# schreibfaul1/ESP32-Opus-Player

Measured on AMD Instinct MI355X. Metric: decoded 48 kHz stereo frames/sec/GPU (x real-time); HBM GB/s vs roofline, higher is better.
Workload: dtype int32 fixed-point (int16/int32 with 64-bit products); 1 GPU; celt_fb_stereo_64k; streams_per_gpu=65536

## Files before the change

esp32-opus-player_amd/csrc/og_celt.hpp:

```cpp
#pragma once
#include "og_celt_bands.hpp"

namespace og {

struct WaveArr {
    typedef RomGlobal Rom;
    OG_MEMBER i32 &pulses(int i) const { return S.pulses_row()[i]; }
    OG_MEMBER i32 &alloc_bits(int i) const { return S.pulses_row()[i]; }
    OG_MEMBER void pulses_rest(int, int) const {}
    OG_MEMBER i32 &fine_quant(int i) const { return S.fine_quant[i]; }
    OG_MEMBER i32 &fine_prio(int i) const { return S.fine_prio[i]; }
    OG_MEMBER i32 &tf_res(int i) const { return S.tf_res[i]; }
    OG_MEMBER void boost_put(int i, int n, int quanta) const { S.offsets[i] = n * quanta; }
    OG_MEMBER i32 boost(int i, int, int) const { return S.offsets[i]; }
    OG_MEMBER i32 &bits1(int i) const { return S.bits1[i]; }
    OG_MEMBER i32 &bits2(int i) const { return S.bits2[i]; }
    OG_MEMBER i16 &bandE(int i) const { return S.bandE_row()[i]; }
    OG_MEMBER void energies_rest() const {}
    OG_MEMBER void energies_back() const {}
};

template <class A, class R>
OG_DEV void coarse_energy(A a, R &rc, int start, int end, int intra, int C, int LM) {
    typedef typename A::Rom T;
    const int pm = (LM * 2 + intra) * 42;
    i32 prev0 = 0, prev1 = 0;
    i32 coef, beta;
    if (intra) {
        coef = 0;
        beta = 4915;
    } else {
        beta = LM == 0 ? 30147 : LM == 1 ? 22282 : LM == 2 ? 12124 : 6554;
        coef = LM == 0 ? 29440 : LM == 1 ? 26112 : LM == 2 ? 21248 : 16384;
    }
    const i32 budget = (i32)rc.storage * 8;
    for (int i = start; i < end; i++) {
        for (int c = 0; c < C; c++) {
            int qi;
            i32 tell = rc_tell(rc);
            if (budget - tell >= 15) {
                int pi = 2 * OG_MIN(i, 20);
                qi = rc_laplace(rc, (u32)T::eprob(pm + pi) << 7, (int)T::eprob(pm + pi + 1) << 6);
            } else if (budget - tell >= 2) {
                u32 s = rc.rng, d = rc.val, r = s >> 2, t;
                int ret = -1;
                do {
                    t = s;
                    ++ret;
                    s = r * (u32)(2 - ret);
                } while (d < s);
                rc.val = d - s;
                rc.rng = t - s;
                rc_renorm(rc);
                qi = (ret >> 1) ^ -(ret & 1);
            } else if (budget - tell >= 1) {
                qi = -rc_bit_logp(rc, 1);
            } else
                qi = -1;
            i32 q = shl32(qi, 10);
            i32 e = OG_MAX(-9 * 1024, (i32)a.bandE(i + c * NBANDS));
            const i32 pv = c ? prev1 : prev0;
            i32 tmp = pshr32(mul16(coef, e), 8) + pv + shl32(q, 7);
            tmp = OG_MAX(-(28 << 17), tmp);
            a.bandE(i + c * NBANDS) = (i16)pshr32(tmp, 7);
            const i32 nv = pv + shl32(q, 7) - mul16(beta, pshr32(q, 8));
            if (c) prev1 = nv; else prev0 = nv;
        }
    }
}

template <class A, class R>
OG_DEV void fine_energy(A a, R &rc, int start, int end, int C) {
    for (int i = start; i < end; i++) {
        int fq = a.fine_quant(i);
        if (fq <= 0) continue;
        for (int c = 0; c < C; c++) {
            i32 q2 = (i32)rc_bits(rc, fq);
            i32 offset = tr16(sub16((shl32(q2, 10) + 512) >> fq, 512));
            a.bandE(i + c * NBANDS) = (i16)(a.bandE(i + c * NBANDS) + offset);
        }
    }
}

template <class A, class R>
OG_DEV void energy_finalise(A a, R &rc, int start, int end, int bits_left, int C) {
    for (int prio = 0; prio < 2; prio++) {
        for (int i = start; i < end && bits_left >= C; i++) {
            if (a.fine_quant(i) >= 8 || a.fine_prio(i) != prio) continue;
            for (int c = 0; c < C; c++) {
                i32 q2 = (i32)rc_bits(rc, 1);
                i32 offset = tr16((shl16(q2, 10) - 512) >> (a.fine_quant(i) + 1));
                a.bandE(i + c * NBANDS) = (i16)(a.bandE(i + c * NBANDS) + offset);
                bits_left--;
            }
        }
    }
}

OG_DEV int tf_select(int LM, int idx) {
    const u32 row0 = 0xF0F0F0F0u, row1 = 0xF101E0F0u, row2 = 0xF102D0E0u, row3 = 0xF103D0E0u;
    u32 row = LM == 0 ? row0 : LM == 1 ? row1 : LM == 2 ? row2 : row3;
    int v = (int)((row >> (4 * idx)) & 15);
    return v >= 8 ? v - 16 : v;
}

template <class A, class R>
OG_DEV void tf_decode(A a, R &rc, int start, int end, int transient, int LM) {
    int curr = 0, tf_sel = 0, tf_changed = 0;
    int logp = transient ? 2 : 4;
    u32 budget = rc.storage * 8, tell = (u32)rc_tell(rc);
    int rsv = LM > 0 && tell + logp + 1 <= budget;
    budget -= rsv;
    for (int i = start; i < end; i++) {
        if (tell + logp <= budget) {
            curr ^= rc_bit_logp(rc, logp);
            tell = (u32)rc_tell(rc);
            tf_changed |= curr;
        }
        a.tf_res(i) = curr;
        logp = transient ? 4 : 5;
    }
    if (rsv && tf_select(LM, 4 * transient + 0 + tf_changed) != tf_select(LM, 4 * transient + 2 + tf_changed))
        tf_sel = rc_bit_logp(rc, 1);
    for (int i = start; i < end; i++) a.tf_res(i) = tf_select(LM, 4 * transient + 2 * tf_sel + a.tf_res(i));
}

template <class T>
OG_DEV i32 celt_band_cap(int j, int LM, int C) {
    const int Nb = (T::eband(j + 1) - T::eband(j)) << LM;
    return (T::pulse_caps(NBANDS * (2 * LM + C - 1) + j) + 64) * C * Nb >> 2;
}

template <class T>
OG_DEV i32 dynalloc_quanta(int j, int LM, int C) {
    const int width = C * (T::eband(j + 1) - T::eband(j)) << LM;
    return OG_MIN(width << BITRES, OG_MAX(6 << BITRES, width));
}

template <class A, class R>
OG_DEV int compute_allocation(A a, R &rc, int start, int end, int alloc_trim, i32 &intensity, i32 &dual_stereo, i32 total,
                               i32 &balance_out, int C, int LM) {
    typedef typename A::Rom T;
    int skip_start = start, intensity_rsv = 0, dual_stereo_rsv = 0;
    OG_STAT(59, total < 0);
    total = OG_MAX(total, 0);
    int skip_rsv = total >= 1 << BITRES ? 1 << BITRES : 0;
    total -= skip_rsv;
    if (C == 2) {
        intensity_rsv = T::log2_frac(end - start);
        if (intensity_rsv > total)
            intensity_rsv = 0;
        else {
            total -= intensity_rsv;
            dual_stereo_rsv = total >= 1 << BITRES ? 1 << BITRES : 0;
// ... 1179 lines not shown
                      const i16 *__restrict__ silk, int silk_n) {
    const i32 t0 = s0 + m;
    m = mul16x32_q15(27853, t0);
    const i32 t1 = s1 + m;
    m = mul16x32_q15(27853, t1);
    const i32 t2 = s2 + m;
    m = mul16x32_q15(27853, t2);
    const i32 t3 = s3 + m;
    m = mul16x32_q15(27853, t3);
#ifdef OG_HOST_EMUL
    const i32 o0 = post_mix(sat16(pshr32(t0, 12)), silk, silk_n, (j + 0) * CC + c), o1 = post_mix(sat16(pshr32(t1, 12)), silk, silk_n, (j + 1) * CC + c);
    const i32 o2 = post_mix(sat16(pshr32(t2, 12)), silk, silk_n, (j + 2) * CC + c), o3 = post_mix(sat16(pshr32(t3, 12)), silk, silk_n, (j + 3) * CC + c);
#else
    const PostAdd ad = post_addends(silk, silk_n, j, c, CC);
    const i32 o0 = sat16(sat16(pshr32(t0, 12)) + ad.a0), o1 = sat16(sat16(pshr32(t1, 12)) + ad.a1);
    const i32 o2 = sat16(sat16(pshr32(t2, 12)) + ad.a2), o3 = sat16(sat16(pshr32(t3, 12)) + ad.a3);
#endif
#ifdef OG_HOST_EMUL
    if (pcm) {
        pcm[(j + 0) * CC + c] = (i16)o0;
        pcm[(j + 1) * CC + c] = (i16)o1;
        pcm[(j + 2) * CC + c] = (i16)o2;
        pcm[(j + 3) * CC + c] = (i16)o3;
    }
#else
    const u32 w01 = (u32)(u16)o0 | (u32)(u16)o1 << 16;
    const u32 w23 = (u32)(u16)o2 | (u32)(u16)o3 << 16;
    og_v2u out;
    int at;
    if (CC == 2) {
        const u32 p01 = (u32)__shfl_xor((int)w01, 1, 64), p23 = (u32)__shfl_xor((int)w23, 1, 64);
        if (c == 0) {
            out.x = (w01 & 0xffffu) | p01 << 16;
            out.y = w01 >> 16 | (p01 & 0xffff0000u);
        } else {
            out.x = (p23 & 0xffffu) | w23 << 16;
            out.y = p23 >> 16 | (w23 & 0xffff0000u);
        }
        at = (j + 2 * c) * 2;
    } else {
        out.x = w01;
        out.y = w23;
        at = j;
    }
    if (pcm) *reinterpret_cast<og_v2u *>(pcm + at) = out;
#endif
}

OG_DEV void celt_post_lane(CeltState *st, int c, int CC, int N, int pos, i16 *__restrict__ pcm, const i16 *__restrict__ silk, int silk_n) {
    const i32 *ring = st->ring[c];
    i32 m = st->deemph[c];
#ifdef OG_HOST_EMUL
    for (int j = 0; j < N; j += 4) {
        const i32 *src = &ring[(pos + j) & RING_MASK];
        celt_post4(m, src[0], src[1], src[2], src[3], j, c, CC, pcm, silk, silk_n);
    }
#else
#define OG_LD4(j) (*reinterpret_cast<const og_v4i *>(&ring[(pos + (j)) & RING_MASK]))
    og_v4i a0 = OG_LD4(0), a1 = OG_LD4(4), a2 = OG_LD4(8), a3 = OG_LD4(12);
    for (int j = 0; j < N; j += 16) {
        const int jn = j + 16 < N ? j + 16 : j;
        const og_v4i b0 = OG_LD4(jn), b1 = OG_LD4(jn + 4), b2 = OG_LD4(jn + 8), b3 = OG_LD4(jn + 12);
        celt_post4(m, a0.x, a0.y, a0.z, a0.w, j, c, CC, pcm, silk, silk_n);
        celt_post4(m, a1.x, a1.y, a1.z, a1.w, j + 4, c, CC, pcm, silk, silk_n);
        celt_post4(m, a2.x, a2.y, a2.z, a2.w, j + 8, c, CC, pcm, silk, silk_n);
        celt_post4(m, a3.x, a3.y, a3.z, a3.w, j + 12, c, CC, pcm, silk, silk_n);
        a0 = b0;
        a1 = b1;
        a2 = b2;
        a3 = b3;
    }
#undef OG_LD4
#endif
    st->deemph[c] = m;
}


OG_DEV void celt_synthesis(CeltState *st, const CeltSynth &p) {
    const int N = p.N, LM = p.LM, C = p.C, CC = p.CC, start = p.start, end = p.end, silence = p.silence, transient = p.transient;
    const int pf_pitch = p.pf_pitch, pf_tapset = p.pf_tapset, M = 1 << LM;
    const i32 pf_gain = p.pf_gain;
    denorm_gains(start, end, C, silence);
    OG_SYNC();
    if (C == 1) {
        OG_FOR_LANES(i, NBANDS) S.bandE_row()[NBANDS + i] = S.bandE_row()[i];
        OG_SYNC();
    }
    if (!p.lost) OG_FOR_LANES(i, 2 * NBANDS) {
        int band = i >= NBANDS ? i - NBANDS : i;
        i32 e = S.bandE_row()[i], l1 = S.logE1_row()[i], l2 = S.logE2_row()[i];
        if (!transient) {
            l2 = l1;
            l1 = e;
        } else
            l1 = OG_MIN(l1, e);
        if (p.loss && !transient) {
            const i32 inc = p.loss->celt_loss_count < 10 ? M : 1024;
            p.loss->backgroundLogE[i] = (i16)OG_MIN((i32)(i16)(p.loss->backgroundLogE[i] + inc), e);
        }
        if (band < start || band >= end) {
            e = 0;
            l1 = l2 = -28 * 1024;
        }
        if (!p.energies_kept_by_parse) st->bandE[i] = (i16)e;
        st->logE1[i] = (i16)l1;
        st->logE2[i] = (i16)l2;
    }
    const int B = transient ? M : 1, shift = transient ? 3 : 3 - LM;
    const int pp = OG_MAX(p.have_state ? p.st_pf_period : st->pf_period, 15), ppo = OG_MAX(p.have_state ? p.st_pf_period_old : st->pf_period_old, 15);
    const i32 pg = p.have_state ? p.st_pf_gain : st->pf_gain, pgo = p.have_state ? p.st_pf_gain_old : st->pf_gain_old;
    const int pt = p.have_state ? p.st_pf_tapset : st->pf_tapset, pto = p.have_state ? p.st_pf_tapset_old : st->pf_tapset_old;
    const int pos = p.have_state ? p.st_ring_pos : st->ring_pos;
    i32 *const SY = syn_buf();
#if defined(OG_RECON_TIGHT) && !defined(OG_HOST_EMUL)
    int touch_code = 0;
    if (!p.lost && LM != 0 && (pgo != 0 || pg != 0 || pf_gain != 0)) {
        const CombRun span = comb_touch_span(comb_touch_plan(ppo, pp, pf_pitch, pgo, pg, pf_gain, pto, pt, pf_tapset, N));
        if (span.lo <= span.hi) touch_code = comb_touch_code(span, pos);
    }
#endif
#ifdef OG_RECON_TIGHT
    for (int c = CC - 1; c >= 0; c--) {
#else
    for (int c = 0; c < CC; c++) {
#endif
        OG_SYNC();
        OG_MARK(14);
#if defined(OG_RECON_TIGHT) && !defined(OG_HOST_EMUL)
        if (!(CC == 1 && C == 2)) denorm_bins((CC == 2 && C == 1) ? 0 : c);
        imdct_channel(st->tail[c], c, N, LM, B, shift, C, CC, st->ring[c], touch_code);
#else
        imdct_channel(st->tail[c], c, N, LM, B, shift, C, CC);
#endif
        OG_MARK(15);
        OG_TAP(2 + 16 * c);
        if (!p.lost) {
            comb_filter(st, c, 0, ppo, pp, 120, pgo, pg, pto, pt, pos);
            if (LM != 0) comb_filter(st, c, 120, pp, pf_pitch, N - 120, pg, pf_gain, pt, pf_tapset, pos);
        }
        OG_TAP(3 + 16 * c);
        OG_SYNC();
        if (p.inline_deemph && OG_LANE == 0) {
            const int plane = pcm_plane(c, C, CC);
            i32 m = st->deemph[c];
            for (int j = 0; j < N; j++) {
                i32 tmp = SY[j] + m;
                m = mul16x32_q15(27853, tmp);
                S.v[plane + j] = (i16)sat16(pshr32(tmp, 12));
            }
            st->deemph[c] = m;
        }
        OG_SYNC();
        OG_MARK(16);
        OG_FOR_LANES(i, N) st->ring[c][(pos + i) & RING_MASK] = SY[i];
        OG_FOR_LANES(i, OVERLAP / 2) st->tail[c][i] = SY[N + i];
    }
    OG_SYNC();
    if (OG_LANE == 0 && p.lost) {
        st->ring_pos = (pos + N) & RING_MASK;
        st->rng = p.rng_final;
        p.loss->celt_loss_count += 1;
    } else if (OG_LANE == 0) {
        if (p.loss) p.loss->celt_loss_count = 0;
        st->ring_pos = (pos + N) & RING_MASK;
        st->rng = p.rng_final;
        int new_old_period = pp, new_old_tapset = pt;
        i32 new_old_gain = pg;
        if (LM != 0) {
            new_old_period = pf_pitch;
            new_old_gain = pf_gain;
            new_old_tapset = pf_tapset;
        }
        st->pf_period_old = new_old_period;
        st->pf_gain_old = new_old_gain;
        st->pf_tapset_old = new_old_tapset;
        st->pf_period = pf_pitch;
        st->pf_gain = pf_gain;
        st->pf_tapset = pf_tapset;
        if (p.rc_error) st->error = 1;
    }
}

OG_DEV int celt_decode_frame(CeltState *st, Rc &rc, int frame_size, int C, int CC, int start, int disable_inv, int end = NBANDS,
                             LossState *loss = nullptr) {
    const i32 *eb = rom_eband;
    int LM;
    for (LM = 0; LM <= 3; LM++)
        if (120 << LM == frame_size) break;
    if (LM > 3) return CELT_BAD_ARG;
    const int M = 1 << LM, N = M * 120;
    if (rc.storage > 1275 || rc.storage <= 1) return CELT_BAD_ARG;

    OG_SYNC();
    OG_FOR_LANES(i, 2 * NBANDS) {
        S.bandE_row()[i] = st->bandE[i];
        S.logE1_row()[i] = st->logE1[i];
        S.logE2_row()[i] = st->logE2[i];
    }
    OG_FOR_LANES(i, 2 * NBANDS) S.cmask_row()[i] = 0;
    OG_FOR_LANES(i, NBANDS) {
        S.pulses_row()[i] = 0;
        S.fine_quant[i] = 0;
        S.fine_prio[i] = 0;
        S.offsets[i] = 0;
    }
    OG_FOR_LANES(i, 2 * N) S.v[V_X + i] = 0;
    OG_FOR_LANES(i, 1248) S.v[V_NORM + i] = 0;
    OG_SYNC();
    if (C == 1) {
        OG_FOR_LANES(i, NBANDS) S.bandE_row()[i] = OG_MAX(S.bandE_row()[i], S.bandE_row()[NBANDS + i]);
        OG_SYNC();
    }

    CeltHeader h;
    celt_parse_header(WaveArr(), rc, start, end, C, LM, h);
    const int silence = h.silence, transient = h.transient, spread = h.spread, pf_pitch = h.pf_pitch, pf_tapset = h.pf_tapset;
    const i32 pf_gain = h.pf_gain, intensity = h.intensity, dual_stereo = h.dual_stereo, balance = h.balance;
    OG_MARK(26);
    const int shortBlocks = transient ? M : 0, anti_collapse_rsv = h.anti_collapse_rsv, codedBands = h.codedBands;
    u32 seed = st->rng;
    decode_all_bands(rc, start, end, C, N, shortBlocks, spread, dual_stereo, intensity,
                     (i32)rc.storage * (8 << BITRES) - anti_collapse_rsv, balance, LM, codedBands, seed, disable_inv);
    OG_MARK(27);
    int anti_collapse_on = 0;
    if (anti_collapse_rsv > 0) anti_collapse_on = (int)rc_bits(rc, 1);
    energy_finalise(WaveArr(), rc, start, end, (i32)rc.storage * 8 - rc_tell(rc), C);
    if (anti_collapse_on) anti_collapse(LM, C, N, start, end, seed);
    if (silence)
        for (int i = 0; i < C * NBANDS; i++) S.bandE_row()[i] = (i16)(-28 * 1024);

    OG_TAP(1);
    CeltSynth sp;
    sp.N = N; sp.LM = LM; sp.C = C; sp.CC = CC; sp.start = start; sp.end = end; sp.silence = silence; sp.transient = transient;
    sp.pf_pitch = pf_pitch; sp.pf_tapset = pf_tapset; sp.pf_gain = pf_gain; sp.rng_final = rc.rng; sp.rc_error = rc.error; sp.inline_deemph = 1;
    sp.loss = loss; sp.lost = 0;
    celt_synthesis(st, sp);
    if (rc_tell(rc) > 8 * (i32)rc.storage) return INTERNAL_ERROR;
    return frame_size;
}

OG_DEV int celt_decode_lost(CeltState *st, LossState *loss, int frame_size, int CC, int start, int end) {
    const i32 *eb = rom_eband;
    int LM;
    for (LM = 0; LM <= 3; LM++)
        if (120 << LM == frame_size) break;
    if (LM > 3) return BAD_ARG;
    const int N = 120 << LM, effEnd = OG_MAX(start, OG_MIN(end, NBANDS));
    const i32 decay = loss->celt_loss_count == 0 ? 1536 : 512;
    OG_SYNC();
    OG_FOR_LANES(i, 2 * NBANDS) {
        const int c = i >= NBANDS, band = i - c * NBANDS;
        i32 e = st->bandE[i];
        if (c < CC && band >= start && band < end) {
            e = OG_MAX((i32)loss->backgroundLogE[i], (i32)(i16)(e - decay));
            st->bandE[i] = (i16)e;
        }
        S.bandE_row()[i] = (i16)e;
    }
    OG_FOR_LANES(i, 2 * N) S.v[V_X + i] = 0;
    OG_SYNC();
    u32 seed = st->rng;
    const int lo = eb[start] << LM, width = (eb[effEnd] << LM) - lo;
    for (int c = 0; c < CC; c++) {
        OG_FOR_LANES(j, width) S.v[V_X + c * N + lo + j] = (i16)((i32)lcg_skip(seed, (u32)j + 1) >> 20);
        seed = lcg_skip(seed, (u32)width);
        for (int i = start; i < effEnd; i++) renormalise(V_X + c * N + (eb[i] << LM), (eb[i + 1] - eb[i]) << LM, 32767);
    }
    CeltSynth sp;
    sp.N = N; sp.LM = LM; sp.C = CC; sp.CC = CC; sp.start = start; sp.end = effEnd; sp.silence = 0; sp.transient = 0;
    sp.pf_pitch = 0; sp.pf_tapset = 0; sp.pf_gain = 0; sp.rng_final = seed; sp.rc_error = 0; sp.inline_deemph = 1;
    sp.loss = loss; sp.lost = 1;
    celt_synthesis(st, sp);
    return frame_size;
}

}

#undef OG_SYNC
#define OG_SYNC() OG_FULL_SYNC()
```

esp32-opus-player_amd/csrc/og_celt_recon_pm.hpp:

```cpp
#pragma once

namespace og {

struct PmLds {
    u32 jdesc[2 * NBANDS];
    u32 jaux[2 * NBANDS];
    u32 bw0[NBANDS], bw1[NBANDS], bw2[NBANDS];
    i32 scale[NBANDS];
    u32 mpar[NBANDS][2];
    u16 jcm[2 * NBANDS];
    u8 binband[100], binoff[100];
};
#ifdef OG_RECON_TIGHT
constexpr int V_PART = V_IY;
static_assert(sizeof(PmLds) <= sizeof(i16) * (V_IY - V_NORM) && 800 <= sizeof(i16) * (V_WIN - V_IY), "the phase-major tables");
#else
constexpr int V_PART = V_NORM + 600;
static_assert(sizeof(PmLds) <= sizeof(i16) * 600 && 600 + 400 <= 1248, "the phase-major tables overlay the folding-history rows");
#endif
OG_DEV PmLds &PM() { return *reinterpret_cast<PmLds *>(&S.v[V_NORM]); }
typedef i32 PmPart[2];
OG_DEV PmPart *pm_part() { return reinterpret_cast<PmPart *>(&S.v[V_PART]); }

enum {
    JD_VALID = 1, JD_FILL = 2,
    JD_PERM_SHIFT = 2 , JD_HAD = 1 << 5,
    JD_STEP_SHIFT = 8
};

struct V8 { i32 v[8]; };
OG_DEV V8 ld8(int pos) {
    V8 r;
#ifdef OG_HOST_EMUL
    for (int k = 0; k < 8; k++) r.v[k] = S.v[pos + k];
#else
    const og_v4i p = *reinterpret_cast<const og_v4i *>(&S.v[pos]);
    r.v[0] = (i32)(i16)p.x; r.v[1] = p.x >> 16; r.v[2] = (i32)(i16)p.y; r.v[3] = p.y >> 16;
    r.v[4] = (i32)(i16)p.z; r.v[5] = p.z >> 16; r.v[6] = (i32)(i16)p.w; r.v[7] = p.w >> 16;
#endif
    return r;
}
OG_DEV void st8(int pos, const V8 &r) {
#ifdef OG_HOST_EMUL
    for (int k = 0; k < 8; k++) S.v[pos + k] = (i16)r.v[k];
#else
    og_v4i p;
    p.x = (i32)(((u32)r.v[0] & 0xffffu) | (u32)r.v[1] << 16); p.y = (i32)(((u32)r.v[2] & 0xffffu) | (u32)r.v[3] << 16);
    p.z = (i32)(((u32)r.v[4] & 0xffffu) | (u32)r.v[5] << 16); p.w = (i32)(((u32)r.v[6] & 0xffffu) | (u32)r.v[7] << 16);
    *reinterpret_cast<og_v4i *>(&S.v[pos]) = p;
#endif
}
OG_DEV void haar_pair(i32 &a, i32 &b) {
    const i32 t1 = mul16(23170, a), t2 = mul16(23170, b);
    a = tr16(pshr32(t1 + t2, 15));
    b = tr16(pshr32(t1 - t2, 15));
}
template <int S_>
OG_DEV void haar8(V8 &r) {
#pragma unroll
    for (int i = 0; i < 8; i++)
        if (!(i & S_)) haar_pair(r.v[i], r.v[i + S_]);
}

struct PmGrp { int band, job, x, gj, N; u32 jd; };
constexpr int PM_GROUPS = 100;
OG_DEV PmGrp pm_group(int g) {
    const PmLds &P = PM();
    PmGrp r;
    const int ch = g >= PM_GROUPS, bin = g - PM_GROUPS * ch;
    r.band = P.binband[bin];
    r.gj = P.binoff[bin];
    r.job = 2 * r.band + ch;
    r.jd = P.jdesc[r.job];
    r.x = V_X + 960 * ch + 8 * (bin - r.gj);
    r.N = (int)(P.bw1[r.band] >> 22) & 255;
    return r;
}

OG_DEV u32 pm_setup_jobs(const ParseRec *rec, int C, int B, u32 &fill_lo, u32 &fill_hi, int &dual_end, int start = 0, bool bw_staged = false) {
    PmLds &P = PM();
    OG_LSYNC();
    OG_FOR_LANES(bin, PM_GROUPS) {
        P.binband[bin] = rom_bin2band[bin];
        P.binoff[bin] = rom_binoff[bin];
    }
    OG_FOR_LANES(i, 2 * NBANDS) {
        P.jdesc[i] = 0;
        P.jcm[i] = 0;
    }
    OG_LSYNC();
    u32 tfm = 0, flo = 0, fhi = 0, de = 0;
    const int logBf = ilog2(B);
    OG_FOR_LANES(l, 2 * NBANDS) {
        const int band = l >> 1, jb = l & 1, coded = band >= start;
#ifdef OG_RECON_TIGHT
        const int bw = !coded ? 0 : bw_staged ? (int)S.band_w_row()[band] : (int)rec->band_w[band];
#else
        const int bw = coded ? (int)rec->band_w[band] : 0;
#endif
        const u32 *wp = rec->words + bw;
        const u32 w0 = coded ? wp[0] : 0u, w1 = coded ? wp[1] : 0u, w2 = coded ? wp[2] : 0u, w3 = coded ? wp[3] : 0u, jw0 = coded ? wp[4] : 0u;
        const int N = (int)(w1 >> 22) & 255;
        const int stereo = (w0 & BW_STEREO) != 0, dual = (w0 & BW_DUAL) != 0, mid_first = (w0 & BW_MID_FIRST) != 0;
        const int njobs = !coded ? 0 : (stereo || dual) ? 2 : 1;
        if (jb == 0) {
            P.bw0[band] = w0;
            P.bw1[band] = w1;
            P.bw2[band] = w2;
            P.scale[band] = (i32)(i16)(w3 & 0xffff);
            if (w0 & BW_DUAL_END) de |= 1u << band;
        }
        const int exists = jb < njobs;
        const int ch = dual ? jb : stereo ? (((jb == 0) == mid_first) ? 0 : 1) : 0;
        const int jpos = bw + 4 + (jb ? 1 + 2 * (int)(jw0 & 31) : 0);
        u32 jw = jw0;
        if (jb && exists) jw = rec->words[OG_MIN(jpos, REC_WORDS_CAP - 1)];
        const int n_fill = (int)(jw & 31), n_pvq = (int)(jw >> JW_NPVQ_SHIFT) & 31;
        P.jaux[l] = (u32)jpos | (u32)ch << 16 | (u32)exists << 17 | (u32)(exists && n_fill > 0) << 18 | (u32)(n_pvq > 0) << 19;
        if (exists) {
            int tf_change = (int)((w0 >> BW_TF_SHIFT) & 7) - 4;
            int recombine = tf_change > 0 ? tf_change : 0, time_divide = 0;
            int logB = logBf - recombine, N_B = (N >> logBf) << recombine;
            while ((N_B & 1) == 0 && tf_change < 0) {
                logB++;
                N_B >>= 1;
                time_divide++;
                tf_change++;
            }
            const int logB0 = logB;
            u32 jd = JD_VALID;
            if (logB0 > 0) jd |= (u32)(logB0 + recombine) << JD_PERM_SHIFT | (B == 1 ? JD_HAD : 0);
            int step = 0;
            for (int k = 0; k < time_divide; k++, step++) jd |= (u32)(logB0 - 1 - k + 1) << (JD_STEP_SHIFT + 4 * step);
            for (int k = 0; k < recombine; k++, step++) jd |= (u32)(k + 1) << (JD_STEP_SHIFT + 4 * step);
            if (n_fill > 0) {
                jd |= JD_FILL;
                if (l < 32) flo |= 1u << l; else fhi |= 1u << (l - 32);
            } else {
                if (logB0 > 0) tfm |= 1u;
                for (int k = 0; k < 3; k++) {
                    const int c = (int)(jd >> (JD_STEP_SHIFT + 4 * k)) & 15;
                    if (c) tfm |= 1u << (1 + 4 * k + (c - 1));
                }
                u32 cm = n_pvq ? S.job_mask_row()[l] : 0u;
                for (int k = 0; k < time_divide; k++) {
                    logB--;
                    cm |= cm >> (1 << logB);
                }
                for (int k = 0; k < recombine; k++) {
                    const u32 c4 = cm & 0xF;
                    cm = ((c4 & 1) * 0x03) | ((c4 >> 1 & 1) * 0x0C) | ((c4 >> 2 & 1) * 0x30) | ((c4 >> 3 & 1) * 0xC0);
                }
                logB += recombine;
                P.jcm[2 * band + ch] = (u16)(cm & ((1u << (1 << logB)) - 1));
            }
            P.jdesc[2 * band + ch] = jd;
        }
    }
    tfm = wave_or(tfm);
    fill_lo = wave_or(flo);
    fill_hi = wave_or(fhi);
    de = wave_or(de);
    dual_end = de ? ilog2((i32)de) : NBANDS + 1;
    OG_LSYNC();
    return tfm;
}

OG_DEV void pm_tf_undo(u32 tfm) {
    constexpr int NG = (2 * PM_GROUPS + OG_NLANES - 1) / OG_NLANES;
    if (tfm & 1u) {
        V8 hold[NG];
        u8 mark[NG];
#pragma unroll
        for (int it = 0; it < NG; it++) {
            const int g = OG_LANE + it * OG_NLANES;
            mark[it] = 0;
            if (g < 2 * PM_GROUPS) {
                const PmGrp q = pm_group(g);
                const int ls = (int)(q.jd >> JD_PERM_SHIFT) & 7;
                if ((q.jd & JD_VALID) && !(q.jd & JD_FILL) && ls) {
                    const int stride = 1 << ls, n0 = q.N >> ls, had = (q.jd & JD_HAD) != 0;
#pragma unroll
                    for (int k = 0; k < 8; k++) {
                        const int inter = 8 * q.gj + k, j = inter >> ls, i = inter & (stride - 1);
                        hold[it].v[k] = S.v[q.x + (had ? ordery(stride, i) : i) * n0 + j];
                    }
                    mark[it] = 1;
                }
            }
        }
        OG_LSYNC();
#pragma unroll
        for (int it = 0; it < NG; it++) {
            const int g = OG_LANE + it * OG_NLANES;
            if (mark[it]) {
                const PmGrp q = pm_group(g);
                st8(q.x + 8 * q.gj, hold[it]);
            }
        }
        OG_LSYNC();
    }
    if (tfm & (1u << (1 + 3))) {
#pragma unroll
        for (int it = 0; it < NG; it++) {
            const int g = OG_LANE + it * OG_NLANES;
            if (g < 2 * PM_GROUPS) {
                const PmGrp q = pm_group(g);
                if ((q.jd & JD_VALID) && !(q.jd & JD_FILL) && ((q.jd >> JD_STEP_SHIFT) & 15) == 4 && !(q.gj & 1)) {
                    V8 a = ld8(q.x + 8 * q.gj), b = ld8(q.x + 8 * q.gj + 8);
#pragma unroll
                    for (int k = 0; k < 8; k++) haar_pair(a.v[k], b.v[k]);
                    st8(q.x + 8 * q.gj, a);
                    st8(q.x + 8 * q.gj + 8, b);
                }
            }
        }
        OG_LSYNC();
    }
    if (tfm & 0x0eeeu) {
#pragma unroll
        for (int it = 0; it < NG; it++) {
            const int g = OG_LANE + it * OG_NLANES;
            if (g < 2 * PM_GROUPS) {
                const PmGrp q = pm_group(g);
                const u32 steps = (q.jd & JD_VALID) && !(q.jd & JD_FILL) ? (q.jd >> JD_STEP_SHIFT) & 0xfffu : 0u;
                if (steps & 0x777u) {
                    V8 r = ld8(q.x + 8 * q.gj);
                    for (int k = 0; k < 3; k++) {
                        const int c = (int)(steps >> (4 * k)) & 15;
                        if (c == 1) haar8<1>(r);
                        else if (c == 2) haar8<2>(r);
                        else if (c == 3) haar8<4>(r);
                    }
                    st8(q.x + 8 * q.gj, r);
                }
            }
        }
        OG_LSYNC();
    }
}

OG_DEV void pm_make_lowband(int dst, int p0, int n, int i, int use_y, int dual_end, int norm_offset = 0, int dup_n1 = 0, int dup_back = 0) {
    const PmLds &P = PM();
    OG_LSYNC();
    OG_FOR_LANES(j, n) {
        int r = p0 + j;
        const bool copied = dup_back && r >= dup_n1;
        if (copied) r -= dup_back;
        const int p = norm_offset + r, sb = P.binband[p >> 3];
        const i32 sc = P.scale[sb];
        i32 v;
        if (i >= dual_end && sb < dual_end && !copied)
            v = ((i32)(i16)mul16_q15(sc, S.v[V_X + p]) + (i32)(i16)mul16_q15(sc, S.v[V_X + 960 + p])) >> 1;
        else
            v = mul16_q15(sc, S.v[V_X + (use_y ? 960 : 0) + p]);
        S.v[dst + j] = (i16)v;
    }
    OG_LSYNC();
}

OG_DEV u32 pm_band_cm(int b, int c) {
    const PmLds &P = PM();
    const u32 w0 = (u32)OG_UNI(P.bw0[b]);
    if (w0 & BW_STEREO) return (u32)OG_UNI(P.jcm[2 * b]) | (u32)OG_UNI(P.jcm[2 * b + 1]);
    return (u32)OG_UNI(P.jcm[2 * b + ((w0 & BW_DUAL) ? c : 0)]);
}

OG_DEV void pm_fill_jobs(const u32 *words, const LcgTab &lcg, u32 fill_lo, u32 fill_hi, int C, int B, int dual_end, u32 &seed,
                         int start = 0) {
    const int norm_offset = 8 * rom_eband[start];
    const int dup_n1 = 8 * (rom_eband[start + 1] - rom_eband[start]), dup_n2 = 8 * (rom_eband[start + 2] - rom_eband[start + 1]);
    PmLds &P = PM();
    RecCur cur;
    cur.words = words;
    cur.w = 0;
    cur.base = -64;
    cur.leaf = 0;
    for (int l = 0; l < 2 * NBANDS; l++) {
        if (!((l < 32 ? fill_lo >> l : fill_hi >> (l - 32)) & 1u)) continue;
        OG_MARK(5);
        OG_STAT(20, 1);
        const int i = l >> 1, jb = l & 1;
        const u32 aux = (u32)OG_UNI(P.jaux[l]), w0 = (u32)OG_UNI(P.bw0[i]), w1 = (u32)OG_UNI(P.bw1[i]);
        const int ch = (int)(aux >> 16) & 1;
        const int eb0 = (int)(w1 >> 11) & 2047, N = (int)(w1 >> 22) & 255;
        const int tf_change = (int)((w0 >> BW_TF_SHIFT) & 7) - 4;
        const int stereo = (w0 & BW_STEREO) != 0, dual = (w0 & BW_DUAL) != 0;
        u32 x_cm, y_cm;
        if (w0 & BW_HAS_LOW) {
            const int fold_end = (int)(w0 >> BW_FOLD1_SHIFT) & 31;
            int fold_i = (int)(w0 >> BW_FOLD0_SHIFT) & 31;
            x_cm = y_cm = 0;
            do {
                x_cm |= pm_band_cm(fold_i, 0);
                y_cm |= pm_band_cm(fold_i, C - 1);
            } while (++fold_i < fold_end);
        } else
            x_cm = y_cm = (1u << B) - 1;
        i32 jfill;
        int want_low;
        if (dual) {
            jfill = (i32)(jb ? y_cm : x_cm);
            want_low = 1;
        } else {
            i32 fill0 = (i32)(x_cm | y_cm);
            if (stereo) {
                if (w0 & BW_THETA0) fill0 &= (1 << B) - 1;
                if (w0 & BW_THETA1) fill0 &= ((1 << B) - 1) << B;
            }
            jfill = ch ? fill0 >> B : fill0;
            want_low = !ch;
        }
        if (jfill == 0 && !(OG_UNI(P.jaux[l]) >> 19 & 1)) {
            OG_STAT(24, 1);
            continue;
        }
        cur.w = (int)(aux & 0xffff);
        OG_STAT(27, 1);
        const u32 jw = rec_word(cur);
        int low = -1;
        if ((w0 & BW_HAS_LOW) && want_low && (jw & JW_NEED_LOW)) {
            const int dup = (i == start + 1 && dup_n2 > dup_n1) ? dup_n2 - dup_n1 : 0;
            pm_make_lowband(V_IY, (int)(w1 & 2047), N, i, dual && ch, dual_end, norm_offset, dup_n1, dup);
            low = V_IY;
        }
        const u32 cm = recon_band_mono(cur, jw, lcg, tf_change, seed, V_X + 960 * ch + eb0, N, B, low, -1, 0, -1, jfill, l);
        if (OG_LANE == 0) P.jcm[2 * i + ch] = (u16)cm;
        OG_LSYNC();
    }
}

OG_DEV void pm_stereo_merge(int C) {
    PmLds &P = PM();
    if (C != 2) return;
    OG_LSYNC();
    const int eb_lo = rom_eband[OG_MIN(OG_LANE, NBANDS - 1)], eb_hi = rom_eband[OG_MIN(OG_LANE, NBANDS - 1) + 1];
    OG_FOR_LANES(g, PM_GROUPS) {
        const int band = P.binband[g];
        if (P.bw0[band] & BW_STEREO) {
            const V8 a = ld8(V_X + 8 * g), b = ld8(V_X + 960 + 8 * g);
            i32 xp = 0, side = 0;
#pragma unroll
            for (int k = 0; k < 8; k++) {
                xp += mul16(b.v[k], a.v[k]);
                side += mul16(b.v[k], b.v[k]);
            }
            pm_part()[g][0] = xp;
            pm_part()[g][1] = side;
        }
    }
    OG_LSYNC();
    OG_FOR_LANES(band, NBANDS) {
        const u32 w0 = P.bw0[band];
        if (w0 & BW_STEREO) {
            const int g0 = OG_NLANES > 1 ? eb_lo : rom_eband[band], g1 = OG_NLANES > 1 ? eb_hi : rom_eband[band + 1];
            i32 xp = 0, side = 0;
            for (int g = g0; g < g1; g++) {
                xp += pm_part()[g][0];
                side += pm_part()[g][1];
            }
            const i32 mid = (i32)(i16)(P.bw2[band] & 0xffff);
            xp = mul16x32_q15(mid, xp);
            const i32 mid2 = tr16(mid >> 1);
            const i32 El = mul16(mid2, mid2) + side - 2 * xp, Er = mul16(mid2, mid2) + side + 2 * xp;
            i32 mode = 1, lgain = 0, rgain = 0;
            int kl = 0, kr = 0;
            if (Er < 161061 || El < 161061)
                mode = 2;
            else {
                kl = ilog2(El) >> 1;
                kr = ilog2(Er) >> 1;
                lgain = rsqrt_norm(vshr32(El, (kl - 7) << 1));
                rgain = rsqrt_norm(vshr32(Er, (kr - 7) << 1));
                if (kl < 7) kl = 7;
                if (kr < 7) kr = 7;
            }
            if (w0 & BW_INV) mode |= 4;
            P.mpar[band][0] = (u32)(mode | kl << 8 | kr << 16);
            P.mpar[band][1] = ((u32)lgain & 0xffffu) | (u32)rgain << 16;
        } else
            P.mpar[band][0] = 0u;
    }
    OG_LSYNC();
    OG_FOR_LANES(g, PM_GROUPS) {
        const int band = P.binband[g];
        const i32 m0 = (i32)P.mpar[band][0];
        if (m0 & 3) {
            const u32 m1 = P.mpar[band][1];
            const i32 lgain = (i32)(i16)(m1 & 0xffff), rgain = (i32)m1 >> 16, mid = (i32)(i16)(P.bw2[band] & 0xffff);
            const int kl = (m0 >> 8) & 255, kr = (m0 >> 16) & 255;
            V8 a = ld8(V_X + 8 * g), b = ld8(V_X + 960 + 8 * g);
#pragma unroll
            for (int k = 0; k < 8; k++) {
                i32 xo, yo;
                if (m0 & 2) {
                    xo = a.v[k];
                    yo = a.v[k];
                } else {
                    const i32 l = tr16(mul16_p15(mid, a.v[k])), r = b.v[k];
                    xo = tr16(pshr32(mul16(lgain, sub16(l, r)), kl + 1));
                    yo = tr16(pshr32(mul16(rgain, add16(l, r)), kr + 1));
                }
                a.v[k] = xo;
                b.v[k] = (m0 & 4) ? tr16(-yo) : yo;
            }
            if (!(m0 & 2)) st8(V_X + 8 * g, a);
            st8(V_X + 960 + 8 * g, b);
        }
    }
    OG_LSYNC();
}

OG_DEV void recon_all_bands_pm(const ParseRec *rec, LcgTab &lcg, int C, int shortBlocks, u32 &seed_io, int start = 0, bool bw_staged = false) {
    const int B = shortBlocks ? 8 : 1;
    u32 fill_lo, fill_hi, seed = seed_io;
    int dual_end;
    OG_MARK(3);
    const u32 tfm = pm_setup_jobs(rec, C, B, fill_lo, fill_hi, dual_end, start, bw_staged);
    if (fill_lo | fill_hi) lcg.hold();
#if defined(OG_HOST_EMUL) && defined(OG_STATS)
    {
        int n_fill_jobs = 0, w_prev = -1;
        bool close_pair = false;
        for (int l = 0; l < 2 * NBANDS; l++)
            if ((l < 32 ? fill_lo >> l : fill_hi >> (l - 32)) & 1u) {
                const int w = (int)(PM().jaux[l] & 0xffff);
                close_pair |= w_prev >= 0 && w - w_prev < 64;
                w_prev = w;
                n_fill_jobs++;
            }
        OG_STAT(33, n_fill_jobs == 0);
        OG_STAT(34, n_fill_jobs == 1);
        OG_STAT(35, n_fill_jobs >= 4);
        OG_STAT(36, close_pair);
    }
#endif
    OG_STAT(0, 1);
    OG_STAT(19, shortBlocks != 0);
    OG_STAT(21, tfm != 0);
    OG_STAT(22, (tfm & 1u) != 0);
    OG_STAT(23, (fill_lo | fill_hi) != 0);
    OG_MARK(8);
    if (tfm) pm_tf_undo(tfm);
    if (fill_lo | fill_hi) pm_fill_jobs(rec->words, lcg, fill_lo, fill_hi, C, B, dual_end, seed, start);
    OG_MARK(10);
    pm_stereo_merge(C);
    OG_MARK(4);
    OG_FOR_LANES(t, NBANDS * C) {
        const PmLds &P = PM();
        const int b = t / C, c = t - b * C;
        const u32 w0 = P.bw0[b];
        const u32 cm = (w0 & BW_STEREO) ? (u32)P.jcm[2 * b] | (u32)P.jcm[2 * b + 1] : (u32)P.jcm[2 * b + ((w0 & BW_DUAL) ? c : 0)];
        S.cmask_row()[t] = (u8)cm;
    }
    OG_LSYNC();
    seed_io = seed;
}

#ifdef OG_RECON_TIGHT
static_assert(sizeof(i32) * 2 * PM_GROUPS <= offsetof(PmLds, binband), "the groups' sums end before the bin tables");
static_assert(48 + 2 * 2 * NBANDS <= 200 && (V_TMP + 48) % 2 == 0, "r and the entries' words fit the scratch row");
OG_DEV void anti_collapse_pm(const LcgTab &lcg, int LM, int C, int size, int start, int end, u32 seed) {
    const PmLds &P = PM();
    const i16 *const rrow = anti_collapse_r(LM, C, start, end);
    u32 *const ent = reinterpret_cast<u32 *>(&S.v[V_TMP + 48]);
    i32 *const part = reinterpret_cast<i32 *>(&S.v[V_NORM]);
    const int NE = C * NBANDS;
    OG_STAT(32, 1);
    u32 run = 0;
    (void)run;
    OG_FOR_LANES(e, OG_NLANES > 1 ? OG_NLANES : NE) {
        const int i = C == 2 ? e >> 1 : e;
        int draws = 0;
        if (e < NE && i >= start && i < end) {
            const int cnt = __builtin_popcount(~(u32)S.cmask_row()[e] & 0xffu);
            draws = cnt * (rom_eband[i + 1] - rom_eband[i]);
            OG_STAT(30, cnt);
            OG_STAT(31, cnt != 0);
        }
#ifdef OG_HOST_EMUL
        const u32 before = run;
        run += (u32)draws;
#else
        const u32 before = (u32)(wave_scan_add(draws) - draws);
#endif
        if (e < NE) ent[e] = lcg_skip(seed, before);
    }
    OG_LSYNC();
    OG_FOR_LANES(t, C * PM_GROUPS) {
        const int c = t >= PM_GROUPS, g = t - PM_GROUPS * c;
        const int i = P.binband[g], j = P.binoff[g], e = i * C + c;
        const u32 clr = (i >= start && i < end) ? ~(u32)S.cmask_row()[e] & 0xffu : 0u;
        if (clr) {
            const int N0 = rom_eband[i + 1] - rom_eband[i];
            const i32 r = rrow[c * NBANDS + i];
            const u32 base = ent[e];
            V8 x = ld8(V_X + c * size + 8 * g);
            int at = j;
            i32 ss = 0;
#pragma unroll
            for (int k = 0; k < 8; k++) {
                const u32 s = lcg.at(base, at);
                if ((clr >> k) & 1u) {
                    x.v[k] = (i16)((s & 0x8000) ? r : -r);
                    at += N0;
                }
                ss += mul16(x.v[k], x.v[k]);
            }
            st8(V_X + c * size + 8 * g, x);
            part[t] = ss;
        }
    }
    OG_LSYNC();
    OG_FOR_LANES(e, NE) {
        const int i = C == 2 ? e >> 1 : e, c = e - i * C;
        u32 w = 0;
        if (i >= start && i < end && (~(u32)S.cmask_row()[e] & 0xffu)) {
            const int g0 = rom_eband[i], g1 = rom_eband[i + 1];
            i32 E = 1;
            for (int g = g0; g < g1; g++) E += part[c * PM_GROUPS + g];
            const int k = ilog2(E) >> 1;
            const i32 t = vshr32(E, 2 * (k - 7));
            const i32 gn = tr16(mul16_p15(rsqrt_norm(t), 32767));
            w = ((u32)gn & 0xffffu) | (u32)((k + 1) & 63) << 16 | 1u << 31;
        }
        ent[e] = w;
    }
    OG_LSYNC();
    OG_FOR_LANES(t, C * PM_GROUPS) {
        const int c = t >= PM_GROUPS, g = t - PM_GROUPS * c;
        const u32 w = ent[P.binband[g] * C + c];
        if (w) {
            const i32 gn = (i32)(i16)(w & 0xffff);
            const int sh = (int)(w >> 16) & 63;
            V8 x = ld8(V_X + c * size + 8 * g);
#pragma unroll
            for (int k = 0; k < 8; k++) x.v[k] = (i16)pshr32(mul16(gn, x.v[k]), sh);
            st8(V_X + c * size + 8 * g, x);
        }
    }
    OG_LSYNC();
}
#endif

}
```

Before: 48.96 million frames/s.

## Add packed int16x2 paths for TF undo, stereo merge and ring stores

After: 50.39 million frames/s (median of 6 runs). 1.03x the previous value.

```diff
diff --git a/esp32-opus-player_amd/csrc/og_celt.hpp b/esp32-opus-player_amd/csrc/og_celt.hpp
--- a/esp32-opus-player_amd/csrc/og_celt.hpp
+++ b/esp32-opus-player_amd/csrc/og_celt.hpp
@@ -1,5 +1,6 @@
 #pragma once
 #include "og_celt_bands.hpp"
+#include "og_celt_packed.hpp"
 
 namespace og {
 
@@ -1485,8 +1486,15 @@
         }
         OG_SYNC();
         OG_MARK(16);
+#if defined(OG_RECON_TIGHT) && !defined(OG_HOST_EMUL)
+        pk_ring_tail_store(st->ring[c], st->tail[c], SY, pos, N);
+#else
+        OG_STAT(61, (pos & 7) != 0);
+        OG_STAT(62, pos + N > RING);
+        OG_STAT(63, 1);
         OG_FOR_LANES(i, N) st->ring[c][(pos + i) & RING_MASK] = SY[i];
         OG_FOR_LANES(i, OVERLAP / 2) st->tail[c][i] = SY[N + i];
+#endif
     }
     OG_SYNC();
     if (OG_LANE == 0 && p.lost) {
diff --git a/esp32-opus-player_amd/csrc/og_celt_packed.hpp b/esp32-opus-player_amd/csrc/og_celt_packed.hpp
--- /dev/null
+++ b/esp32-opus-player_amd/csrc/og_celt_packed.hpp
@@ -0,0 +1,182 @@
+#pragma once
+#include <stddef.h>
+#include "og_celt_bands.hpp"
+
+namespace og {
+
+#if defined(OG_RECON_TIGHT) && !defined(OG_HOST_EMUL)
+constexpr bool PM_PACKED = true;
+#else
+constexpr bool PM_PACKED = false;
+#endif
+
+#ifdef OG_HOST_EMUL
+OG_DEV u32 pk_perm(u32 hi, u32 lo, u32 sel) {
+    const u64 v = (u64)hi << 32 | lo;
+    u32 r = 0;
+    for (int b = 0; b < 4; b++) r |= (u32)((v >> (8 * ((sel >> (8 * b)) & 7u))) & 0xffu) << (8 * b);
+    return r;
+}
+OG_DEV i32 pk_dot2(u32 a, u32 b, i32 acc) {
+    return (i32)((u32)acc + (u32)((i32)(i16)a * (i32)(i16)b) + (u32)(((i32)a >> 16) * ((i32)b >> 16)));
+}
+OG_DEV i32 pk_dot2_fits(u32 a, u32 b, i32 acc) { return pk_dot2(a, b, acc); }
+OG_DEV u32 pk_add16(u32 a, u32 b) { return ((a + b) & 0xffffu) | ((a & 0xffff0000u) + (b & 0xffff0000u)); }
+OG_DEV u32 pk_sub16(u32 a, u32 b) { return ((a - b) & 0xffffu) | ((a & 0xffff0000u) - (b & 0xffff0000u)); }
+#else
+typedef unsigned short og_u16x2 __attribute__((ext_vector_type(2)));
+OG_DEV u32 pk_perm(u32 hi, u32 lo, u32 sel) { return __builtin_amdgcn_perm(hi, lo, sel); }
+OG_DEV i32 pk_dot2(u32 a, u32 b, i32 acc) { return rs_dot2(a, b, acc); }
+OG_DEV i32 pk_dot2_fits(u32 a, u32 b, i32 acc) {
+    return __builtin_amdgcn_sdot2(__builtin_bit_cast(og_i16x2, a), __builtin_bit_cast(og_i16x2, b), acc, true);
+}
+OG_DEV u32 pk_add16(u32 a, u32 b) { return __builtin_bit_cast(u32, __builtin_bit_cast(og_u16x2, a) + __builtin_bit_cast(og_u16x2, b)); }
+OG_DEV u32 pk_sub16(u32 a, u32 b) { return __builtin_bit_cast(u32, __builtin_bit_cast(og_u16x2, a) - __builtin_bit_cast(og_u16x2, b)); }
+#endif
+OG_DEV u32 pk_lolo(u32 a, u32 b) { return pk_perm(b, a, 0x05040100u); }
+OG_DEV u32 pk_hihi(u32 a, u32 b) { return pk_perm(b, a, 0x07060302u); }
+OG_DEV u32 pk_pair(i32 lo, i32 hi) { return ((u32)lo & 0xffffu) | (u32)hi << 16; }
+OG_DEV u32 pk_q15(i32 lo, i32 hi) { return (((u32)lo >> 15) & 0xffffu) | (((u32)hi << 1) & 0xffff0000u); }
+OG_DEV u32 pk_shr(i32 lo, i32 hi, int s) { return pk_pair(lo >> s, hi >> s); }
+
+struct W4 { u32 w[4]; };
+#ifdef OG_HOST_EMUL
+template <typename T>
+OG_DEV T pk_ld(const i16 *p) {
+    T v;
+    memcpy(&v, p, sizeof(T));
+    return v;
+}
+OG_DEV W4 ldw4(const i16 *p) { return pk_ld<W4>(p); }
+OG_DEV void stw4(i16 *p, const W4 &r) { memcpy(p, &r, sizeof(r)); }
+#else
+typedef i32 og_v4i __attribute__((ext_vector_type(4)));
+template <typename T>
+OG_DEV T pk_ld(const i16 *p) { return *reinterpret_cast<const T *>(p); }
+OG_DEV W4 ldw4(const i16 *p) {
+    const og_v4i v = *reinterpret_cast<const og_v4i *>(p);
+    return W4{{(u32)v.x, (u32)v.y, (u32)v.z, (u32)v.w}};
+}
+OG_DEV void stw4(i16 *p, const W4 &r) { *reinterpret_cast<og_v4i *>(p) = og_v4i{(i32)r.w[0], (i32)r.w[1], (i32)r.w[2], (i32)r.w[3]}; }
+#endif
+
+#ifdef OG_HOST_EMUL
+struct W2 { u32 w[2]; };
+#else
+struct alignas(8) W2 { u32 w[2]; };
+#endif
+
+constexpr u32 HAAR_SUM = 23170u | 23170u << 16, HAAR_DIF = 23170u | (u32)(u16)(-23170) << 16;
+OG_DEV void pk_haar_words(u32 &x, u32 &y) {
+    const u32 p = pk_lolo(x, y), q = pk_hihi(x, y);
+    x = pk_q15(pk_dot2_fits(p, HAAR_SUM, 16384), pk_dot2_fits(q, HAAR_SUM, 16384));
+    y = pk_q15(pk_dot2_fits(p, HAAR_DIF, 16384), pk_dot2_fits(q, HAAR_DIF, 16384));
+}
+OG_DEV void pk_haar8_1(W4 &r) {
+    i32 s[4], d[4];
+#pragma unroll
+    for (int m = 0; m < 4; m++) {
+        s[m] = pk_dot2_fits(r.w[m], HAAR_SUM, 16384);
+        d[m] = pk_dot2_fits(r.w[m], HAAR_DIF, 16384);
+    }
+#pragma unroll
+    for (int m = 0; m < 4; m++) r.w[m] = pk_q15(s[m], d[m]);
+}
+OG_DEV void pk_haar8_2(W4 &r) { pk_haar_words(r.w[0], r.w[1]); pk_haar_words(r.w[2], r.w[3]); }
+OG_DEV void pk_haar8_4(W4 &r) { pk_haar_words(r.w[0], r.w[2]); pk_haar_words(r.w[1], r.w[3]); }
+OG_DEV void pk_haar16(W4 &a, W4 &b) {
+#pragma unroll
+    for (int m = 0; m < 4; m++) pk_haar_words(a.w[m], b.w[m]);
+}
+
+static_assert(V_X % 8 == 0 && 960 % 8 == 0, "a channel's spectrum starts 16-byte aligned, its bands at multiples of 8 coefficients");
+OG_DEV W4 pk_gather(const i16 *x, int N, int gj, int ls, bool had) {
+    W4 r;
+    if (ls == 2) {
+        const int n0 = N >> 2;
+        const i16 *p = x + 2 * gj;
+        const u32 r0 = pk_ld<u32>(p + (had ? 3 : 0) * n0), r1 = pk_ld<u32>(p + (had ? 0 : 1) * n0);
+        const u32 r2 = pk_ld<u32>(p + 2 * n0), r3 = pk_ld<u32>(p + (had ? 1 : 3) * n0);
+        r.w[0] = pk_lolo(r0, r1);
+        r.w[1] = pk_lolo(r2, r3);
+        r.w[2] = pk_hihi(r0, r1);
+        r.w[3] = pk_hihi(r2, r3);
+    } else if (ls == 3) {
+        const int n0 = N >> 3;
+        const i16 *p = x + gj;
+        const u32 rows = had ? 0x25163407u : 0x76543210u;
+#pragma unroll
+        for (int m = 0; m < 4; m++)
+            r.w[m] = (u32)pk_ld<u16>(p + (int)((rows >> (8 * m)) & 15u) * n0) | (u32)pk_ld<u16>(p + (int)((rows >> (8 * m + 4)) & 15u) * n0) << 16;
+    } else if (ls == 1) {
+        const int n0 = N >> 1;
+        const i16 *p = x + 4 * gj;
+        const W2 a = pk_ld<W2>(p + (had ? n0 : 0)), b = pk_ld<W2>(p + (had ? 0 : n0));
+        r.w[0] = pk_lolo(a.w[0], b.w[0]);
+        r.w[1] = pk_hihi(a.w[0], b.w[0]);
+        r.w[2] = pk_lolo(a.w[1], b.w[1]);
+        r.w[3] = pk_hihi(a.w[1], b.w[1]);
+    } else {
+        const int stride = 1 << ls, n0 = N >> ls;
+        i32 v[8];
+#pragma unroll
+        for (int k = 0; k < 8; k++) {
+            const int inter = 8 * gj + k, j = inter >> ls, i = inter & (stride - 1);
+            v[k] = x[(had ? ordery(stride, i) : i) * n0 + j];
+        }
+#pragma unroll
+        for (int m = 0; m < 4; m++) r.w[m] = pk_pair(v[2 * m], v[2 * m + 1]);
+    }
+    return r;
+}
+
+OG_DEV void pk_merge_sums(const W4 &a, const W4 &b, i32 &xp, i32 &side) {
+#pragma unroll
+    for (int m = 0; m < 4; m++) {
+        xp = pk_dot2(b.w[m], a.w[m], xp);
+        side = pk_dot2(b.w[m], b.w[m], side);
+    }
+}
+OG_DEV void pk_merge_apply(W4 &a, W4 &b, i32 mid, i32 lgain, i32 rgain, int kl, int kr, bool inv) {
+    const u32 m_lo = (u32)mid & 0xffffu, m_hi = (u32)mid << 16;
+    const u32 l_lo = (u32)lgain & 0xffffu, l_hi = (u32)lgain << 16, r_lo = (u32)rgain & 0xffffu, r_hi = (u32)rgain << 16;
+    const i32 rl = (1 << (kl + 1)) >> 1, rr = (1 << (kr + 1)) >> 1;
+#pragma unroll
+    for (int m = 0; m < 4; m++) {
+        const u32 l = pk_q15(pk_dot2_fits(a.w[m], m_lo, 16384), pk_dot2_fits(a.w[m], m_hi, 16384));
+        const u32 d = pk_sub16(l, b.w[m]), s = pk_add16(l, b.w[m]);
+        a.w[m] = pk_shr(pk_dot2_fits(d, l_lo, rl), pk_dot2_fits(d, l_hi, rl), kl + 1);
+        const u32 y = pk_shr(pk_dot2_fits(s, r_lo, rr), pk_dot2_fits(s, r_hi, rr), kr + 1);
+        b.w[m] = inv ? pk_sub16(0u, y) : y;
+    }
+}
+OG_DEV W4 pk_neg(const W4 &a) { return W4{{pk_sub16(0u, a.w[0]), pk_sub16(0u, a.w[1]), pk_sub16(0u, a.w[2]), pk_sub16(0u, a.w[3])}}; }
+
+static_assert(RING % 8 == 0 && 120 % 8 == 0 && OVERLAP / 2 % 4 == 0, "ring pieces of 4 samples: whole, and never across the wrap");
+static_assert(offsetof(CeltState, ring) % 16 == 0 && offsetof(CeltState, tail) % 16 == 0 && sizeof(CeltState) % 16 == 0 &&
+              sizeof(((CeltState *)nullptr)->tail[0]) % 16 == 0, "the ring and the tails are 16-byte aligned");
+static_assert(V_SYN % 8 == 0, "the synthesis buffer is 16-byte aligned in the working set");
+struct P4 { i32 v[4]; };
+OG_DEV P4 pk_ld4(const i32 *p) {
+#ifdef OG_HOST_EMUL
+    P4 r;
+    memcpy(&r, p, sizeof(r));
+    return r;
+#else
+    const og_v4i v = *reinterpret_cast<const og_v4i *>(p);
+    return P4{{v.x, v.y, v.z, v.w}};
+#endif
+}
+OG_DEV void pk_st4(i32 *p, const P4 &r) {
+#ifdef OG_HOST_EMUL
+    memcpy(p, &r, sizeof(r));
+#else
+    *reinterpret_cast<og_v4i *>(p) = og_v4i{r.v[0], r.v[1], r.v[2], r.v[3]};
+#endif
+}
+OG_DEV void pk_ring_tail_store(i32 *ring, i32 *tail, const i32 *sy, int pos, int n) {
+    OG_FOR_LANES(p, n / 4) pk_st4(&ring[(pos + 4 * p) & RING_MASK], pk_ld4(&sy[4 * p]));
+    OG_FOR_LANES(p, OVERLAP / 2 / 4) pk_st4(&tail[4 * p], pk_ld4(&sy[n + 4 * p]));
+}
+
+}
diff --git a/esp32-opus-player_amd/csrc/og_celt_recon_pm.hpp b/esp32-opus-player_amd/csrc/og_celt_recon_pm.hpp
--- a/esp32-opus-player_amd/csrc/og_celt_recon_pm.hpp
+++ b/esp32-opus-player_amd/csrc/og_celt_recon_pm.hpp
@@ -61,6 +61,9 @@
     for (int i = 0; i < 8; i++)
         if (!(i & S_)) haar_pair(r.v[i], r.v[i + S_]);
 }
+
+template <bool PACKED> struct PmHold { typedef V8 type; };
+template <> struct PmHold<true> { typedef W4 type; };
 
 struct PmGrp { int band, job, x, gj, N; u32 jd; };
 constexpr int PM_GROUPS = 100;
@@ -166,10 +169,12 @@
     return tfm;
 }
 
+template <bool PACKED = PM_PACKED>
 OG_DEV void pm_tf_undo(u32 tfm) {
     constexpr int NG = (2 * PM_GROUPS + OG_NLANES - 1) / OG_NLANES;
+    typedef typename PmHold<PACKED>::type Hold;
     if (tfm & 1u) {
-        V8 hold[NG];
+        Hold hold[NG];
         u8 mark[NG];
 #pragma unroll
         for (int it = 0; it < NG; it++) {
@@ -180,10 +185,14 @@
                 const int ls = (int)(q.jd >> JD_PERM_SHIFT) & 7;
                 if ((q.jd & JD_VALID) && !(q.jd & JD_FILL) && ls) {
                     const int stride = 1 << ls, n0 = q.N >> ls, had = (q.jd & JD_HAD) != 0;
-#pragma unroll
-                    for (int k = 0; k < 8; k++) {
-                        const int inter = 8 * q.gj + k, j = inter >> ls, i = inter & (stride - 1);
-                        hold[it].v[k] = S.v[q.x + (had ? ordery(stride, i) : i) * n0 + j];
+                    if constexpr (PACKED)
+                        hold[it] = pk_gather(&S.v[q.x], q.N, q.gj, ls, had);
+                    else {
+#pragma unroll
+                        for (int k = 0; k < 8; k++) {
+                            const int inter = 8 * q.gj + k, j = inter >> ls, i = inter & (stride - 1);
+                            hold[it].v[k] = S.v[q.x + (had ? ordery(stride, i) : i) * n0 + j];
+                        }
                     }
                     mark[it] = 1;
                 }
@@ -195,7 +204,8 @@
             const int g = OG_LANE + it * OG_NLANES;
             if (mark[it]) {
                 const PmGrp q = pm_group(g);
-                st8(q.x + 8 * q.gj, hold[it]);
+                if constexpr (PACKED) stw4(&S.v[q.x + 8 * q.gj], hold[it]);
+                else st8(q.x + 8 * q.gj, hold[it]);
             }
         }
         OG_LSYNC();
@@ -207,11 +217,18 @@
             if (g < 2 * PM_GROUPS) {
                 const PmGrp q = pm_group(g);
                 if ((q.jd & JD_VALID) && !(q.jd & JD_FILL) && ((q.jd >> JD_STEP_SHIFT) & 15) == 4 && !(q.gj & 1)) {
-                    V8 a = ld8(q.x + 8 * q.gj), b = ld8(q.x + 8 * q.gj + 8);
-#pragma unroll
-                    for (int k = 0; k < 8; k++) haar_pair(a.v[k], b.v[k]);
-                    st8(q.x + 8 * q.gj, a);
-                    st8(q.x + 8 * q.gj + 8, b);
+                    if constexpr (PACKED) {
+                        W4 a = ldw4(&S.v[q.x + 8 * q.gj]), b = ldw4(&S.v[q.x + 8 * q.gj + 8]);
+                        pk_haar16(a, b);
+                        stw4(&S.v[q.x + 8 * q.gj], a);
+                        stw4(&S.v[q.x + 8 * q.gj + 8], b);
+                    } else {
+                        V8 a = ld8(q.x + 8 * q.gj), b = ld8(q.x + 8 * q.gj + 8);
+#pragma unroll
+                        for (int k = 0; k < 8; k++) haar_pair(a.v[k], b.v[k]);
+                        st8(q.x + 8 * q.gj, a);
+                        st8(q.x + 8 * q.gj + 8, b);
+                    }
                 }
             }
         }
@@ -225,14 +242,25 @@
                 const PmGrp q = pm_group(g);
                 const u32 steps = (q.jd & JD_VALID) && !(q.jd & JD_FILL) ? (q.jd >> JD_STEP_SHIFT) & 0xfffu : 0u;
                 if (steps & 0x777u) {
-                    V8 r = ld8(q.x + 8 * q.gj);
-                    for (int k = 0; k < 3; k++) {
-                        const int c = (int)(steps >> (4 * k)) & 15;
-                        if (c == 1) haar8<1>(r);
-                        else if (c == 2) haar8<2>(r);
-                        else if (c == 3) haar8<4>(r);
+                    if constexpr (PACKED) {
+                        W4 r = ldw4(&S.v[q.x + 8 * q.gj]);
+                        for (int k = 0; k < 3; k++) {
+                            const int c = (int)(steps >> (4 * k)) & 15;
+                            if (c == 1) pk_haar8_1(r);
+                            else if (c == 2) pk_haar8_2(r);
+                            else if (c == 3) pk_haar8_4(r);
+                        }
+                        stw4(&S.v[q.x + 8 * q.gj], r);
+                    } else {
+                        V8 r = ld8(q.x + 8 * q.gj);
+                        for (int k = 0; k < 3; k++) {
+                            const int c = (int)(steps >> (4 * k)) & 15;
+                            if (c == 1) haar8<1>(r);
+                            else if (c == 2) haar8<2>(r);
+                            else if (c == 3) haar8<4>(r);
+                        }
+                        st8(q.x + 8 * q.gj, r);
                     }
-                    st8(q.x + 8 * q.gj, r);
                 }
             }
         }
@@ -330,6 +358,7 @@
     }
 }
 
+template <bool PACKED = PM_PACKED>
 OG_DEV void pm_stereo_merge(int C) {
     PmLds &P = PM();
     if (C != 2) return;
@@ -338,12 +367,17 @@
     OG_FOR_LANES(g, PM_GROUPS) {
         const int band = P.binband[g];
         if (P.bw0[band] & BW_STEREO) {
-            const V8 a = ld8(V_X + 8 * g), b = ld8(V_X + 960 + 8 * g);
+            OG_STAT(29, 1);
             i32 xp = 0, side = 0;
-#pragma unroll
-            for (int k = 0; k < 8; k++) {
-                xp += mul16(b.v[k], a.v[k]);
-                side += mul16(b.v[k], b.v[k]);
+            if constexpr (PACKED)
+                pk_merge_sums(ldw4(&S.v[V_X + 8 * g]), ldw4(&S.v[V_X + 960 + 8 * g]), xp, side);
+            else {
+                const V8 a = ld8(V_X + 8 * g), b = ld8(V_X + 960 + 8 * g);
+#pragma unroll
+                for (int k = 0; k < 8; k++) {
+                    xp += mul16(b.v[k], a.v[k]);
+                    side += mul16(b.v[k], b.v[k]);
+                }
             }
             pm_part()[g][0] = xp;
             pm_part()[g][1] = side;
@@ -389,23 +423,37 @@
             const u32 m1 = P.mpar[band][1];
             const i32 lgain = (i32)(i16)(m1 & 0xffff), rgain = (i32)m1 >> 16, mid = (i32)(i16)(P.bw2[band] & 0xffff);
             const int kl = (m0 >> 8) & 255, kr = (m0 >> 16) & 255;
-            V8 a = ld8(V_X + 8 * g), b = ld8(V_X + 960 + 8 * g);
-#pragma unroll
-            for (int k = 0; k < 8; k++) {
-                i32 xo, yo;
-                if (m0 & 2) {
-                    xo = a.v[k];
-                    yo = a.v[k];
-                } else {
-                    const i32 l = tr16(mul16_p15(mid, a.v[k])), r = b.v[k];
-                    xo = tr16(pshr32(mul16(lgain, sub16(l, r)), kl + 1));
-                    yo = tr16(pshr32(mul16(rgain, add16(l, r)), kr + 1));
-                }
-                a.v[k] = xo;
-                b.v[k] = (m0 & 4) ? tr16(-yo) : yo;
-            }
-            if (!(m0 & 2)) st8(V_X + 8 * g, a);
-            st8(V_X + 960 + 8 * g, b);
+            OG_STAT(37, 1);
+            OG_STAT(38, (m0 & 2) != 0);
+            if constexpr (PACKED) {
+                W4 a = ldw4(&S.v[V_X + 8 * g]), b;
+                if (m0 & 2)
+                    b = (m0 & 4) ? pk_neg(a) : a;
+                else {
+                    b = ldw4(&S.v[V_X + 960 + 8 * g]);
+                    pk_merge_apply(a, b, mid, lgain, rgain, kl, kr, (m0 & 4) != 0);
+                    stw4(&S.v[V_X + 8 * g], a);
+                }
+                stw4(&S.v[V_X + 960 + 8 * g], b);
+            } else {
+                V8 a = ld8(V_X + 8 * g), b = ld8(V_X + 960 + 8 * g);
+#pragma unroll
+                for (int k = 0; k < 8; k++) {
+                    i32 xo, yo;
+                    if (m0 & 2) {
+                        xo = a.v[k];
+                        yo = a.v[k];
+                    } else {
+                        const i32 l = tr16(mul16_p15(mid, a.v[k])), r = b.v[k];
+                        xo = tr16(pshr32(mul16(lgain, sub16(l, r)), kl + 1));
+                        yo = tr16(pshr32(mul16(rgain, add16(l, r)), kr + 1));
+                    }
+                    a.v[k] = xo;
+                    b.v[k] = (m0 & 4) ? tr16(-yo) : yo;
+                }
+                if (!(m0 & 2)) st8(V_X + 8 * g, a);
+                st8(V_X + 960 + 8 * g, b);
+            }
         }
     }
     OG_LSYNC();
@@ -433,6 +481,28 @@
         OG_STAT(34, n_fill_jobs == 1);
         OG_STAT(35, n_fill_jobs >= 4);
         OG_STAT(36, close_pair);
+    }
+    {
+        OG_STAT(25, (tfm & (1u << 4)) != 0);
+        OG_STAT(28, (tfm & 0x0eeeu) != 0);
+        for (int l = 0; l < 2 * NBANDS; l++) {
+            const u32 jd = PM().jdesc[l];
+            const int groups = (int)((PM().bw1[l >> 1] >> 22) & 255) / 8;
+            if (!(jd & JD_VALID) || !(jd & ~(u32)(JD_VALID | JD_FILL))) continue;
+            if (jd & JD_FILL) {
+                OG_STAT(60, groups);
+                continue;
+            }
+            const u32 steps = (jd >> JD_STEP_SHIFT) & 0xfffu;
+            const int ls = (int)(jd >> JD_PERM_SHIFT) & 7, had = (jd & JD_HAD) != 0;
+            OG_STAT(ls == 2 && had && steps == 0x012u ? 39
+                    : ls == 3 && had && steps == 0x123u ? 43
+                    : ls == 0 && steps == 0x321u ? 47
+                    : ls == 3 && !had && steps == 0x001u ? 48
+                    : ls == 3 && !had && steps == 0u ? 49
+                    : ls == 4 && !had && steps == 0x004u ? 54
+                    : 55, groups);
+        }
     }
 #endif
     OG_STAT(0, 1);
```
